# ratschlab/secedo

Measured on NVIDIA B200. Metric: similarity-matrix significant loci/s (8K cells, 0.5x), higher is better.
Workload: dtype int8 tensor-core counts (int32 accumulate) + f64 log-likelihood epilogue

## Files before the change

secedo_b200/csrc/common.cuh:

```cuda
#pragma once

#include <cuda_runtime.h>

#include <atomic>
#include <cstdarg>
#include <cstdint>
#include <cstdio>
#include <deque>
#include <map>
#include <string>
#include <unordered_map>
#include <vector>

#include "../../include/secedo_b200.h"

struct sgpu_ctx {
    int device = 0;
    int sm_count = 148;
    cudaStream_t own_stream = nullptr;
    cudaStream_t stream = nullptr;
    cudaStream_t copy_stream = nullptr;
    cudaStream_t d2h_stream = nullptr;
    cudaEvent_t out_done = nullptr;
    void *pending_out = nullptr;
// ... 199 lines not shown
    uint64_t slab_t0 = 0, slab_t1 = 0, slab_raw_tiles = 0;
    uint32_t slab_nb = 0;
    double *slab_raw = nullptr;
    unsigned long long *slab_minmax = nullptr;
    double *slab_out = nullptr;
};

constexpr uint32_t CODE_DROPPED = 0xFFFFFFFFu;
__host__ __device__ inline uint32_t code_cell(uint32_t c) { return c >> 4; }
__host__ __device__ inline uint32_t code_base(uint32_t c) { return (c >> 2) & 3u; }
__host__ __device__ inline bool code_tail(uint32_t c) { return (c >> 1) & 1u; }
__host__ __device__ inline bool code_multi(uint32_t c) { return c & 1u; }

struct LinkResult {
    DevBuf<uint32_t> sp_bits;
    DevBuf<uint64_t> sp_rank;
    DevBuf<uint32_t> sp_entry;
    DevBuf<uint32_t> sp_locus;
    DevBuf<uint32_t> sp_start;
    DevBuf<uint32_t> sp_head;
    DevBuf<uint32_t> sp_code;
    DevBuf<uint8_t> sp_drop;
    DevBuf<uint32_t> sp_rcode;
    DevBuf<uint64_t> g_off;
    DevBuf<uint32_t> g_list;
    DevBuf<uint8_t> g_base;
    DevBuf<uint32_t> g_nst;
    uint64_t n_special = 0;
    DevBuf<uint64_t> me_idx;
    DevBuf<uint32_t> me_code;
    DevBuf<uint32_t> me_locus;
    DevBuf<uint32_t> me_pos;
    DevBuf<uint32_t> me_beg;
    DevBuf<uint32_t> me_end;
    DevBuf<uint8_t> lchr;
    DevBuf<uint64_t> tail_locus;
    std::vector<uint64_t> h_tail_locus;
    DevBuf<uint32_t> tail_loci;
    uint64_t n_tail_loci = 0;
    DevBuf<uint32_t> gmap;
    uint32_t n_groups = 0, num_cells = 0;
    bool gmap_identity = false;
    bool ranged = false;
    DevBuf<uint8_t> owned;
    DevBuf<uint32_t> own_loci;
    uint64_t n_own = 0;
    DevBuf<uint32_t> code;
    uint64_t n_reads = 0, n_multi = 0, n_dropped = 0, n_tail = 0;
    uint64_t n_span_splits = 0;
};

int sgpu_scan_u8_u64(sgpu_ctx *ctx, const uint8_t *in, uint64_t *out, uint64_t n);
int sgpu_scan_u32_u64(sgpu_ctx *ctx, const uint32_t *in, uint64_t *out, uint64_t n);

int sgpu_filter_impl(sgpu_ctx *ctx, const sgpu_pileup *in, const uint32_t *h_id_to_pos, uint32_t n_groups,
                     double theta, int cell_proportion, sgpu_pileup **filtered, double *avg_coverage);
int sgpu_is_significant_impl(sgpu_ctx *ctx, const uint16_t *h_counts4, uint64_t n, double theta,
                             int cell_proportion, uint8_t *h_out);

struct RangeSpec {
    const uint32_t *own_pos_begin, *own_pos_end, *tail_position;
};
struct CutoffQuery {
    const uint8_t *whole;
    uint32_t *tail_position;
    uint8_t *resolved;
};
int sgpu_link_reads(sgpu_ctx *ctx, const sgpu_pileup *p, uint32_t num_cells, uint32_t L,
                    const uint32_t *h_group_id_to_pos, uint32_t n_groups, uint32_t num_threads,
                    LinkResult *out, const RangeSpec *range = nullptr, const CutoffQuery *cutq = nullptr);
int sgpu_cutoff_from_suffix(sgpu_ctx *ctx, const sgpu_pileup *p, uint32_t L, uint32_t num_threads, const uint8_t *h_whole,
                            uint32_t *h_tail_position, uint8_t *h_resolved);
int sgpu_link_dense_codes(sgpu_ctx *ctx, const sgpu_pileup *p, LinkResult *lr);
int sgpu_link_candidates(sgpu_ctx *ctx, LinkResult *lr, uint32_t min_nst);

int sgpu_choose_path(const sgpu_pileup *p, uint32_t num_cells);

int sgpu_scatter_pairs(sgpu_ctx *ctx, const sgpu_pileup *p, const LinkResult &lr, sgpu_counts *c,
                       int sign, bool only_tail_pairs, uint64_t *n_pairs);

int sgpu_multilocus(sgpu_ctx *ctx, const sgpu_pileup *p, LinkResult &lr, sgpu_counts *c,
                    uint32_t L, uint64_t *n_pairs_multi);

struct FTable {
    double F[SGPU_MAX_CLASS * SGPU_MAX_CLASS];
};
int sgpu_log_probs_impl(sgpu_ctx *ctx, double eps, double h, double theta, uint32_t L, uint32_t n,
                        double *h_ls, double *h_ld);
int sgpu_epilogue(sgpu_ctx *ctx, sgpu_counts *c, uint32_t L, double eps, double h, double theta,
                  int normalization, double *h_out, double **d_keep = nullptr, bool async_out = false);
int sgpu_output_wait_impl(sgpu_ctx *ctx);
int sgpu_slab_raw_impl(sgpu_ctx *ctx, sgpu_counts *c, const int32_t *const *peer_planes, const double *const *peer_spill,
                       uint32_t n_peers, uint32_t slab, uint32_t n_slabs, uint32_t L, double eps, double h, double theta,
                       double **d_extrema);
int sgpu_slab_finalize_impl(sgpu_ctx *ctx, sgpu_counts *c, int normalization, double *out, double **d_out);

int sgpu_em_impl(sgpu_ctx *ctx, const sgpu_pileup *p, const uint32_t *h_id_to_pos, uint32_t n_groups, double theta,
                 double *h_prob_b, uint32_t n_cells, uint32_t max_iterations, uint32_t *iterations, float *ms_total);

int sgpu_spectral_device(sgpu_ctx *ctx, const double *d_A, uint32_t n, uint32_t k, double tol, double *h_evals,
                         double *h_evecs, sgpu_spectral_stats *stats);
int sgpu_laplacian_device(sgpu_ctx *ctx, const double *d_A, uint32_t n, double *h_out);
int sgpu_spectral_matvec_host(sgpu_ctx *ctx, const double *h_M, uint32_t n, int width, const double *h_X, const double *h_W,
                              double alpha, double beta, double gamma, double *h_out);
int sgpu_build_gtable(sgpu_ctx *ctx, double eps, double h, double theta, uint32_t L, uint32_t n,
                      double *d_G , double *d_F );
// ... 24 lines not shown
```

secedo_b200/csrc/reads.cu:

```cuda
#include "common.cuh"

#include <algorithm>
#include <cstdlib>
#include <vector>

namespace {

constexpr int TB = 256;
constexpr uint64_t KEY_EMPTY = ~0ull;

__device__ __forceinline__ uint64_t mix64(uint64_t x) {
    x ^= x >> 33;
    x *= 0xff51afd7ed558ccdull;
    x ^= x >> 33;
    x *= 0xc4ceb9fe1a85ec53ull;
    x ^= x >> 33;
    return x;
}

__device__ __forceinline__ uint32_t chr_of_locus(const uint64_t *__restrict__ chr_ptr, uint32_t n_chr, uint64_t l) {
    uint32_t lo = 0, hi = n_chr;
    while (hi - lo > 1) {
        uint32_t mid = (lo + hi) >> 1;
        if (chr_ptr[mid] <= l) {
            lo = mid;
        } else {
            hi = mid;
        }
    }
    return lo;
}

__device__ __forceinline__ uint32_t locus_of_entry(const uint64_t *__restrict__ row_ptr, uint64_t n_loci, uint64_t e) {
    uint64_t lo = 0, hi = n_loci;
    while (hi - lo > 1) {
        const uint64_t mid = (lo + hi) >> 1;
        if (row_ptr[mid] <= e) {
            lo = mid;
        } else {
            hi = mid;
        }
    }
    return static_cast<uint32_t>(lo);
}

__global__ void __launch_bounds__(TB) locus_meta_kernel(const uint64_t *__restrict__ row_ptr,
                                                        const uint32_t *__restrict__ position,
                                                        const uint64_t *__restrict__ chr_ptr, uint32_t n_chr,
                                                        uint64_t n_loci, uint8_t *__restrict__ lchr,
                                                        unsigned int *__restrict__ max_row, int *__restrict__ err) {
    const uint64_t l = static_cast<uint64_t>(blockIdx.x) * TB + threadIdx.x;
    unsigned int n = 0;
    if (l < n_loci) {
        const uint32_t c = chr_of_locus(chr_ptr, n_chr, l);
        lchr[l] = static_cast<uint8_t>(c);
        if (l > chr_ptr[c] && position[l] <= position[l - 1]) {
            atomicExch(err, SGPU_E_POSITIONS);
        }
        n = static_cast<unsigned int>(min(row_ptr[l + 1] - row_ptr[l], static_cast<uint64_t>(0xFFFFFFFFu)));
    }
#pragma unroll
    for (int o = 16; o > 0; o >>= 1) {
        n = max(n, __shfl_xor_sync(0xffffffffu, n, o));
    }
    if ((threadIdx.x & 31) == 0 && n) {
        atomicMax(max_row, n);
    }
}

constexpr int WIN_THREADS = 512;
constexpr uint32_t SLOT_EMPTY = 0xFFFFu;
constexpr uint32_t REC_BUF = 1024;
constexpr uint32_t WIN_MAX_ENTRIES = 0xFFFEu;
constexpr size_t WIN_SMEM_LIMIT = 220 * 1024;

struct WinCounters {
    unsigned long long n_links;
};

__device__ __forceinline__ uint32_t slot_hash(uint32_t id, uint32_t shift) { return (id * 0x9E3779B1u) >> shift; }

__device__ __forceinline__ void emit_link(uint2 *rbuf, uint32_t *s_cnt, uint2 *__restrict__ links, uint64_t cap,
                                          WinCounters *__restrict__ ctr, uint32_t x, uint32_t y) {
    const uint32_t k = atomicAdd(s_cnt, 1u);
    if (k < REC_BUF) {
        rbuf[k] = make_uint2(x, y);
    } else {
        const unsigned long long g = atomicAdd(&ctr->n_links, 1ull);
        if (g < cap) {
            links[g] = make_uint2(x, y);
        }
    }
}

__device__ __forceinline__ void cp_async4(void *dst, const void *src) {
    asm volatile("cp.async.ca.shared.global [%0], [%1], 4;" ::"r"(static_cast<uint32_t>(__cvta_generic_to_shared(dst))), "l"(src) : "memory");
}
__device__ __forceinline__ void cp_async16(void *dst, const void *src) {
    asm volatile("cp.async.cg.shared.global [%0], [%1], 16;" ::"r"(static_cast<uint32_t>(__cvta_generic_to_shared(dst))), "l"(src) : "memory");
}
__device__ __forceinline__ void cp_async_commit() { asm volatile("cp.async.commit_group;" ::: "memory"); }
template <int N>
__device__ __forceinline__ void cp_async_wait() {
    asm volatile("cp.async.wait_group %0;" ::"n"(N) : "memory");
}

constexpr uint32_t WIN_RING = 3;
constexpr uint32_t WIN_META = 64;
constexpr uint32_t WIN_META_N = WIN_META + WIN_RING + 1;

__global__ void __launch_bounds__(WIN_THREADS, 2) link_window_kernel(
        const uint64_t *__restrict__ row_ptr, const uint32_t *__restrict__ position, const uint32_t *__restrict__ read_id,
        const uint64_t *__restrict__ src_off ,
        const uint8_t *__restrict__ lchr, uint64_t n_loci, uint32_t L, uint32_t loci_per_cta,
        uint32_t slots , uint32_t id_cap ,
        uint32_t n_ring ,
        uint2 *__restrict__ links, uint64_t cap, WinCounters *__restrict__ ctr) {
    extern __shared__ __align__(16) uint32_t s_mem[];
    uint32_t *ring = s_mem;
    uint2 *rbuf = reinterpret_cast<uint2 *>(s_mem + n_ring * id_cap);
    unsigned short *tab = reinterpret_cast<unsigned short *>(rbuf + REC_BUF);
    __shared__ uint64_t s_row[WIN_META_N + 1];
    __shared__ uint64_t s_src[WIN_META_N];
    __shared__ uint32_t s_pos[WIN_META_N];
    __shared__ uint8_t s_chr[WIN_META_N];
    __shared__ uint32_t s_cnt;
    __shared__ unsigned long long s_base;
    const uint32_t mask = slots - 1, shift = 32 - (31 - __clz(slots));
    const uint64_t la = static_cast<uint64_t>(blockIdx.x) * loci_per_cta;
    const uint64_t lb = min(n_loci, la + loci_per_cta);
    if (threadIdx.x == 0) {
        s_cnt = 0;
    }
    if (la >= lb) {
        return;
    }
    const bool aligned16 = (reinterpret_cast<uintptr_t>(read_id) & 15u) == 0;
    uint64_t meta0 = la;
    auto load_meta = [&](uint64_t base) {
        for (uint32_t i = threadIdx.x; i <= WIN_META_N; i += WIN_THREADS) {
            const uint64_t l = base + i;
            s_row[i] = row_ptr[min(l, n_loci)];
            if (i < WIN_META_N) {
                s_pos[i] = l < n_loci ? position[l] : 0;
                s_chr[i] = l < n_loci ? lchr[l] : 0xFF;
                s_src[i] = l < n_loci ? (src_off ? src_off[l] : row_ptr[l]) : 0;
            }
        }
    };
    auto prefetch = [&](uint64_t l) {
        if (l < n_loci && l - meta0 < WIN_META_N) {
            const uint64_t e0 = s_src[l - meta0];
            uint32_t *dst = ring + (l % n_ring) * id_cap + (e0 & 3u);
            const uint32_t *src = read_id + e0;
            const uint32_t n = static_cast<uint32_t>(s_row[l - meta0 + 1] - s_row[l - meta0]);
            const uint32_t head = aligned16 ? min(n, static_cast<uint32_t>((4 - (e0 & 3u)) & 3u)) : n;
            const uint32_t body = (n - head) >> 2;
            for (uint32_t i = threadIdx.x; i < head; i += WIN_THREADS) {
                cp_async4(dst + i, src + i);
            }
            for (uint32_t i = threadIdx.x; i < body; i += WIN_THREADS) {
                cp_async16(dst + head + 4 * i, src + head + 4 * i);
            }
            const uint32_t done = head + 4 * body;
// ... 192 lines not shown
    }
}

__global__ void __launch_bounds__(TB) ghash_emit_kernel(const uint64_t *__restrict__ row_ptr,
                                                        const uint32_t *__restrict__ read_id,
                                                        const uint8_t *__restrict__ lchr, uint64_t n_loci,
                                                        const uint64_t *__restrict__ keys, const uint32_t *__restrict__ vals,
                                                        uint64_t mask, uint2 *__restrict__ links, uint64_t cap,
                                                        WinCounters *__restrict__ ctr) {
    for (uint64_t l = blockIdx.x; l < n_loci; l += gridDim.x) {
        const uint64_t e0 = row_ptr[l], e1 = row_ptr[l + 1];
        const uint64_t chr = lchr[l];
        for (uint64_t base = e0; base < e1; base += TB) {
            const uint64_t e = base + threadIdx.x;
            uint32_t first = 0xFFFFFFFFu;
            if (e < e1) {
                const uint64_t key = (chr << 32) | read_id[e];
                uint64_t slot = mix64(key) & mask;
                while (keys[slot] != key) {
                    slot = (slot + 1) & mask;
                }
                first = vals[slot];
            }
            const bool hit = e < e1 && first != static_cast<uint32_t>(e);
            const uint32_t ballot = __ballot_sync(0xffffffffu, hit);
            if (ballot) {
                const int lane = threadIdx.x & 31, leader = __ffs(ballot) - 1;
                unsigned long long g = 0;
                if (lane == leader) {
                    g = atomicAdd(&ctr->n_links, static_cast<unsigned long long>(__popc(ballot)));
                }
                g = __shfl_sync(0xffffffffu, g, leader);
                if (hit) {
                    g += __popc(ballot & ((1u << lane) - 1u));
                    if (g < cap) {
                        links[g] = make_uint2(first, static_cast<uint32_t>(e));
                    }
                }
            }
        }
    }
}

__global__ void __launch_bounds__(TB) mark_kernel(const uint2 *__restrict__ links, uint64_t n_links,
                                                  uint32_t *__restrict__ bits) {
    const uint64_t i = static_cast<uint64_t>(blockIdx.x) * TB + threadIdx.x;
    if (i < n_links) {
        const uint2 r = links[i];
        atomicOr(&bits[r.x >> 5], 1u << (r.x & 31));
        atomicOr(&bits[r.y >> 5], 1u << (r.y & 31));
    }
}

__global__ void __launch_bounds__(TB) popc_kernel(const uint32_t *__restrict__ bits, uint64_t n_words,
                                                  uint32_t *__restrict__ pc) {
    const uint64_t w = static_cast<uint64_t>(blockIdx.x) * TB + threadIdx.x;
    if (w < n_words) {
        pc[w] = __popc(bits[w]);
    }
}

__device__ __forceinline__ uint32_t sid_of(const uint32_t *__restrict__ bits, const uint64_t *__restrict__ rank, uint32_t e) {
    return static_cast<uint32_t>(rank[e >> 5]) + __popc(bits[e >> 5] & ((1u << (e & 31)) - 1u));
}

__global__ void __launch_bounds__(TB) word_locus_kernel(const uint64_t *__restrict__ row_ptr, uint64_t n_loci,
                                                        uint64_t n_words, uint32_t *__restrict__ word_locus) {
    const int lane = threadIdx.x & 31;
    const uint64_t warps_total = static_cast<uint64_t>(gridDim.x) * (TB / 32);
    for (uint64_t l = static_cast<uint64_t>(blockIdx.x) * (TB / 32) + (threadIdx.x >> 5); l < n_loci; l += warps_total) {
        const uint64_t e0 = row_ptr[l], e1 = l + 1 < n_loci ? row_ptr[l + 1] : n_words * 32;
        for (uint64_t w = (e0 + 31) / 32 + lane; w * 32 < e1 && w < n_words; w += 32) {
            word_locus[w] = static_cast<uint32_t>(l);
        }
    }
}

__global__ void __launch_bounds__(TB) sp_list_kernel(const uint32_t *__restrict__ bits, const uint64_t *__restrict__ rank,
                                                     uint64_t n_words, const uint64_t *__restrict__ row_ptr,
                                                     const uint32_t *__restrict__ word_locus, uint32_t *__restrict__ sp_entry,
                                                     uint32_t *__restrict__ sp_first, uint32_t *__restrict__ sp_locus) {
    const uint64_t w = static_cast<uint64_t>(blockIdx.x) * TB + threadIdx.x;
    if (w >= n_words) {
        return;
    }
    uint32_t b = bits[w];
    if (b == 0) {
        return;
    }
    uint64_t k = rank[w];
    uint32_t l = word_locus[w];
    uint64_t l_end = row_ptr[l + 1];
    while (b) {
        const uint32_t bit = __ffs(b) - 1;
        b &= b - 1;
        const uint32_t e = static_cast<uint32_t>(w * 32 + bit);
        while (e >= l_end) {
            ++l;
            l_end = row_ptr[l + 1];
        }
        sp_entry[k] = e;
        sp_first[k] = e;
        sp_locus[k] = l;
        ++k;
    }
}

__global__ void __launch_bounds__(TB) link_min_kernel(const uint2 *__restrict__ links, uint64_t n_links,
                                                      const uint32_t *__restrict__ bits, const uint64_t *__restrict__ rank,
                                                      uint32_t *__restrict__ sp_first, int *__restrict__ changed) {
    const uint64_t i = static_cast<uint64_t>(blockIdx.x) * TB + threadIdx.x;
    if (i >= n_links) {
        return;
    }
    const uint2 r = links[i];
    const uint32_t sx = sid_of(bits, rank, r.x), sy = sid_of(bits, rank, r.y);
    const uint32_t fx = sp_first[sx], fy = sp_first[sy];
    const uint32_t m = min(fx, fy);
    if (fx != m) {
        atomicMin(&sp_first[sx], m);
        *changed = 1;
    }
    if (fy != m) {
        atomicMin(&sp_first[sy], m);
// ... 327 lines not shown
        s_multi = 0;
    }
    __syncthreads();
    uint32_t dropped = 0, multi_head = 0;
    for (uint64_t s = static_cast<uint64_t>(blockIdx.x) * TB + threadIdx.x; s < n_special; s += static_cast<uint64_t>(gridDim.x) * TB) {
        const uint32_t h = sp_head[s];
        const uint32_t multi = g_nst[h] >= 2 ? 1u : 0u;
        multi_head += (h == s) & multi;
        const bool drop = sp_drop[s] != 0;
        if (drop) {
            sp_code[s] = CODE_DROPPED;
            ++dropped;
        }
        if (!drop || h == s) {
            const uint32_t gid = gid_base[sp_entry[h]] >> 2;
            uint32_t cell = 0;
            if (gid >= n_groups || (cell = gmap[gid]) >= num_cells) {
                atomicExch(err, SGPU_E_CELL_RANGE);
                cell = 0;
            }
            const uint32_t base = gid_base[sp_entry[s]] & 3u;
            const uint32_t hl = sp_locus[h];
            const uint32_t tail = hl >= tail_locus[lchr[hl]] ? 1u : 0u;
            if (!drop) {
                sp_code[s] = (cell << 4) | (base << 2) | (tail << 1) | multi;
            }
            if (h == s) {
                sp_rcode[s] = (cell << 4) | (tail << 1) | multi;
            }
        }
    }
#pragma unroll
    for (int o = 16; o > 0; o >>= 1) {
        dropped += __shfl_xor_sync(0xffffffffu, dropped, o);
        multi_head += __shfl_xor_sync(0xffffffffu, multi_head, o);
    }
    if ((threadIdx.x & 31) == 0) {
        if (dropped) {
            atomicAdd(&s_dropped, dropped);
        }
        if (multi_head) {
            atomicAdd(&s_multi, multi_head);
        }
    }
    __syncthreads();
    if (threadIdx.x == 0) {
        if (s_dropped) {
            atomicAdd(&stats[0], static_cast<unsigned long long>(s_dropped));
        }
        if (s_multi) {
            atomicAdd(&stats[1], static_cast<unsigned long long>(s_multi));
        }
    }
}

__global__ void __launch_bounds__(TB) sp_start_kernel(const uint32_t *__restrict__ sp_locus, uint64_t n_special,
                                                      uint64_t n_loci, uint32_t *__restrict__ sp_start) {
    const uint64_t l = static_cast<uint64_t>(blockIdx.x) * TB + threadIdx.x;
    if (l > n_loci) {
        return;
    }
    uint64_t lo = 0, hi = n_special;
    while (lo < hi) {
        const uint64_t mid = (lo + hi) >> 1;
        if (sp_locus[mid] < l) {
            lo = mid + 1;
        } else {
            hi = mid;
        }
    }
    sp_start[l] = static_cast<uint32_t>(lo);
}

__global__ void __launch_bounds__(TB) me_flag_kernel(const uint32_t *__restrict__ sp_code, const uint32_t *__restrict__ sp_head,
                                                     const uint32_t *__restrict__ sp_locus, const uint64_t *__restrict__ g_off,
                                                     const uint32_t *__restrict__ g_list, const uint32_t *__restrict__ g_nst,
                                                     uint64_t n_special, uint32_t min_nst, uint32_t *__restrict__ flag,
                                                     uint32_t *__restrict__ pos) {
    const uint64_t s = static_cast<uint64_t>(blockIdx.x) * TB + threadIdx.x;
    if (s >= n_special) {
        return;
    }
    const uint32_t c = sp_code[s];
    uint32_t f = 0;
    if (c != CODE_DROPPED && (c & 1u) && g_nst[sp_head[s]] >= min_nst) {
        const uint32_t h = sp_head[s], loc = sp_locus[s], n = g_nst[h];
        const uint64_t o = g_off[h];
        uint32_t i = 0;
        while (i < n && g_list[o + i] != loc) {
            ++i;
        }
        f = i + 1 < n ? 1u : 0u;
        pos[s] = static_cast<uint32_t>(o + i);
    }
    flag[s] = f;
}

__global__ void __launch_bounds__(TB) me_compact_kernel(const uint32_t *__restrict__ flag, const uint32_t *__restrict__ pos,
                                                        const uint64_t *__restrict__ me_idx, const uint32_t *__restrict__ sp_code,
                                                        const uint32_t *__restrict__ sp_head, const uint32_t *__restrict__ sp_locus,
                                                        const uint64_t *__restrict__ g_off, const uint32_t *__restrict__ g_nst,
                                                        uint64_t n_special, uint32_t *__restrict__ me_code,
                                                        uint32_t *__restrict__ me_locus, uint32_t *__restrict__ me_pos,
                                                        uint32_t *__restrict__ me_beg, uint32_t *__restrict__ me_end) {
    const uint64_t s = static_cast<uint64_t>(blockIdx.x) * TB + threadIdx.x;
    if (s >= n_special || !flag[s]) {
        return;
    }
    const uint64_t k = me_idx[s];
    const uint32_t h = sp_head[s];
    me_code[k] = sp_code[s];
    me_locus[k] = sp_locus[s];
    me_pos[k] = pos[s];
    me_beg[k] = static_cast<uint32_t>(g_off[h]);
    me_end[k] = static_cast<uint32_t>(g_off[h]) + g_nst[h];
}

template <typename GB>
__global__ void __launch_bounds__(TB) dense_codes_kernel(const uint64_t *__restrict__ row_ptr,
                                                         const GB *__restrict__ gid_base,
                                                         const uint8_t *__restrict__ lchr,
                                                         const uint64_t *__restrict__ tail_locus,
                                                         const uint32_t *__restrict__ gmap, uint32_t n_groups,
                                                         uint32_t num_cells, uint64_t n_loci, uint32_t *__restrict__ code,
// ... 64 lines not shown
            SGPU_CUDA(ctx, cudaMemcpyAsync(out->tail_locus.p, p->d_chr_ptr + 1, p->n_chr * sizeof(uint64_t), cudaMemcpyDeviceToDevice, st));
        }
        SGPU_CUDA(ctx, out->tail_loci.alloc(1, ctx));
        return SGPU_OK;
    }

    SGPU_TRACE(ctx, "link: enter");
    DevBuf<int> d_err;
    DevBuf<unsigned int> d_maxn;
    DevBuf<WinCounters> d_ctr;
    DevBuf<unsigned long long> d_stats;
    DevBuf<uint64_t> readbase, n_tail_reads;
    SGPU_CUDA(ctx, d_err.alloc(2, ctx));
    SGPU_CUDA(ctx, d_maxn.alloc(1, ctx));
    SGPU_CUDA(ctx, d_ctr.alloc(1, ctx));
    SGPU_CUDA(ctx, d_stats.alloc(2, ctx));
    SGPU_CUDA(ctx, readbase.alloc(P + 1, ctx));
    SGPU_CUDA(ctx, n_tail_reads.alloc(p->n_chr, ctx));
    SGPU_CUDA(ctx, cudaMemsetAsync(d_err.p, 0, 2 * sizeof(int), st));
    SGPU_CUDA(ctx, cudaMemsetAsync(d_maxn.p, 0, sizeof(unsigned int), st));
    SGPU_CUDA(ctx, cudaMemsetAsync(d_ctr.p, 0, sizeof(WinCounters), st));
    SGPU_CUDA(ctx, cudaMemsetAsync(d_stats.p, 0, 2 * sizeof(unsigned long long), st));

    SGPU_LAUNCH(ctx, (locus_meta_kernel<<<blocks_for(P), TB, 0, st>>>(p->d_row_ptr, p->d_position, p->d_chr_ptr, p->n_chr, P,
                                                                       out->lchr.p, d_maxn.p, d_err.p)));
    uint32_t max_n = p->max_row;
    if (max_n == 0) {
        SGPU_CUDA(ctx, cudaMemcpyAsync(&ctx->h_scratch[0], d_maxn.p, sizeof(unsigned int), cudaMemcpyDeviceToHost, st));
        SGPU_CUDA(ctx, cudaStreamSynchronize(st));
        max_n = static_cast<uint32_t>(ctx->h_scratch[0] & 0xFFFFFFFFu);
        p->max_row = max_n;
    }

    SGPU_TRACE(ctx, "link: allocs+meta");
    const uint32_t id_cap = (max_n + 3 + 3) & ~3u;
    unsigned long long slot_factor = 3;
    if (const char *env = getenv("SECEDO_B200_WIN_SLOT_FACTOR")) {
        slot_factor = static_cast<unsigned long long>(std::max(1, atoi(env)));
    }
    const size_t win_limit = ctx->win_smem_limit ? std::min<size_t>(ctx->win_smem_limit, WIN_SMEM_LIMIT) : WIN_SMEM_LIMIT;
    auto pow2_slots = [&](unsigned long long want) {
        uint32_t sl = 1024;
        while (sl < want && sl < 65536) {
            sl <<= 1;
        }
        return sl;
    };
    uint32_t n_ring = WIN_RING, slots = 1024;
    auto win_smem = [&](uint32_t s) {
        return static_cast<size_t>(n_ring) * id_cap * 4 + REC_BUF * sizeof(uint2) + static_cast<size_t>(s) * 2;
    };
    auto choose_geometry = [&](size_t limit) {
        const uint32_t s_full = pow2_slots(slot_factor * max_n), s_half = std::min(s_full, pow2_slots(2ull * max_n));
        const uint32_t cand[4][2] = { { WIN_RING, s_full }, { 2, s_full }, { WIN_RING, s_half }, { 2, s_half } };
        const char *env_ring = getenv("SECEDO_B200_WIN_RING");
        for (const auto &cd : cand) {
            n_ring = cd[0];
            slots = cd[1];
            if (win_smem(slots) <= limit && !(env_ring && env_ring[0] == '1')) {
                return true;
            }
        }
        n_ring = 1;
        slots = s_full;
        while (slots > 1024 && win_smem(slots) > limit) {
            slots >>= 1;
        }
        return win_smem(slots) <= limit && 4ull * slots >= 5ull * max_n;
    };
    bool window_fits = choose_geometry(win_limit);
    if (!window_fits && win_limit < WIN_SMEM_LIMIT) {
        window_fits = choose_geometry(WIN_SMEM_LIMIT);
    }
    const char *force_global = getenv("SECEDO_B200_FORCE_GLOBAL_HASH");
    const bool use_window = max_n <= WIN_MAX_ENTRIES && window_fits && 4ull * slots >= 5ull * max_n
            && !(force_global && force_global[0] == '1');
    const unsigned locus_grid = static_cast<unsigned>(std::min<uint64_t>(P, static_cast<uint64_t>(ctx->sm_count) * 16));

    DevBuf<uint2> links;
    uint64_t cap = std::max<uint64_t>(E / 8, 4096);
    uint64_t NL = 0;
    for (int attempt = 0; attempt < 2; ++attempt) {
        SGPU_CUDA(ctx, links.alloc(cap, ctx));
        SGPU_CUDA(ctx, cudaMemsetAsync(d_ctr.p, 0, sizeof(WinCounters), st));
        if (use_window) {
            const size_t smem = win_smem(slots);
            SGPU_CUDA(ctx, cudaFuncSetAttribute(link_window_kernel, cudaFuncAttributeMaxDynamicSharedMemorySize, static_cast<int>(smem)));
            const unsigned per_sm = static_cast<unsigned>(std::max<size_t>(1, std::min<size_t>(4, (224 * 1024) / (smem + 2560))));
            const uint64_t want = std::min<uint64_t>(P, static_cast<uint64_t>(ctx->sm_count) * per_sm);
            const uint32_t loci_per_cta = static_cast<uint32_t>(ceil_div_u64(P, want));
            const unsigned wgrid = static_cast<unsigned>(ceil_div_u64(P, loci_per_cta));
            SGPU_TRY(sgpu_cache_preference(ctx, false));
            SGPU_LAUNCH(ctx, (link_window_kernel<<<wgrid, WIN_THREADS, smem, st>>>(p->d_row_ptr, p->d_position,
                                                                                  p->d_read_id ? p->d_read_id : p->view_read_id,
                                                                                  p->d_read_id ? nullptr : p->view_off, out->lchr.p, P, L,
                                                                                  loci_per_cta, slots, id_cap, n_ring, links.p, cap, d_ctr.p)));
        } else {
            SGPU_TRY(sgpu_pileup_materialize(ctx, p));
            DevBuf<uint64_t> keys;
            DevBuf<uint32_t> vals;
            uint64_t hcap = 1024;
            while (hcap < 2 * E) {
                hcap <<= 1;
            }
            SGPU_CUDA(ctx, keys.alloc(hcap, ctx));
            SGPU_CUDA(ctx, vals.alloc(hcap, ctx));
            SGPU_CUDA(ctx, cudaMemsetAsync(keys.p, 0xFF, hcap * sizeof(uint64_t), st));
            SGPU_CUDA(ctx, cudaMemsetAsync(vals.p, 0xFF, hcap * sizeof(uint32_t), st));
            SGPU_LAUNCH(ctx, (ghash_insert_kernel<<<locus_grid, TB, 0, st>>>(p->d_row_ptr, p->d_read_id, out->lchr.p, P, keys.p, vals.p, hcap - 1)));
            SGPU_LAUNCH(ctx, (ghash_emit_kernel<<<locus_grid, TB, 0, st>>>(p->d_row_ptr, p->d_read_id, out->lchr.p, P, keys.p, vals.p, hcap - 1,
                                                                            links.p, cap, d_ctr.p)));
        }
        SGPU_CUDA(ctx, cudaGetLastError());
        if (ctx->flush_point == 0) {
            SGPU_TRY(sgpu_tensor_flush(ctx, true));
        }
        SGPU_CUDA(ctx, cudaMemcpyAsync(&ctx->h_scratch[0], d_ctr.p, sizeof(uint64_t), cudaMemcpyDeviceToHost, st));
        SGPU_CUDA(ctx, cudaStreamSynchronize(st));
        NL = ctx->h_scratch[0];
        if (NL <= cap) {
            break;
        }
        if (attempt == 1) {
            return sgpu_fail(ctx, SGPU_E_CUDA, "link list overflow on retry (%llu > %llu)", (unsigned long long)NL, (unsigned long long)cap);
        }
        cap = NL;
    }

    SGPU_TRACE(ctx, "link: window kernel");
    uint64_t NS = 0;
    DevBuf<uint32_t> nf_locus;
    DevBuf<uint64_t> nf_scan;
    if (NL) {
        DevBuf<uint32_t> pc;
        SGPU_CUDA(ctx, pc.alloc(W, ctx));
        SGPU_CUDA(ctx, out->sp_rank.alloc(W + 1, ctx));
        SGPU_LAUNCH(ctx, (mark_kernel<<<blocks_for(NL), TB, 0, st>>>(links.p, NL, out->sp_bits.p)));
        SGPU_LAUNCH(ctx, (popc_kernel<<<blocks_for(W), TB, 0, st>>>(out->sp_bits.p, W, pc.p)));
        SGPU_TRY(sgpu_scan_u32_u64(ctx, pc.p, out->sp_rank.p, W));
        SGPU_CUDA(ctx, cudaMemcpyAsync(&ctx->h_scratch[0], out->sp_rank.p + W, sizeof(uint64_t), cudaMemcpyDeviceToHost, st));
        SGPU_CUDA(ctx, cudaStreamSynchronize(st));
        NS = ctx->h_scratch[0];
    }
    SGPU_TRACE(ctx, "link: mark+rank");
    out->n_special = NS;
    SGPU_CUDA(ctx, out->sp_start.alloc(P + 1, ctx));
    if (NS == 0) {
        SGPU_CUDA(ctx, cudaMemsetAsync(out->sp_start.p, 0, (P + 1) * sizeof(uint32_t), st));
    }
    DevBuf<uint32_t> sp_first, g_cnt, cursor;
    if (NS) {
        SGPU_CUDA(ctx, out->sp_entry.alloc(NS, ctx));
        SGPU_CUDA(ctx, out->sp_locus.alloc(NS, ctx));
        SGPU_CUDA(ctx, out->sp_head.alloc(NS, ctx));
        SGPU_CUDA(ctx, out->sp_code.alloc(NS, ctx));
        SGPU_CUDA(ctx, out->sp_drop.alloc(NS, ctx));
        SGPU_CUDA(ctx, out->sp_rcode.alloc(NS, ctx));
        SGPU_CUDA(ctx, out->g_off.alloc(NS + 1, ctx));
        SGPU_CUDA(ctx, out->g_list.alloc(NS, ctx));
        SGPU_CUDA(ctx, out->g_base.alloc(NS, ctx));
        SGPU_CUDA(ctx, out->g_nst.alloc(NS, ctx));
        SGPU_CUDA(ctx, sp_first.alloc(NS, ctx));
        SGPU_CUDA(ctx, g_cnt.alloc(NS, ctx));
        SGPU_CUDA(ctx, cursor.alloc(NS, ctx));
        SGPU_CUDA(ctx, nf_locus.alloc(P, ctx));
        SGPU_CUDA(ctx, nf_scan.alloc(P + 1, ctx));
        {
            DevBuf<uint32_t> word_locus;
            SGPU_CUDA(ctx, word_locus.alloc(W, ctx));
            SGPU_LAUNCH(ctx, (word_locus_kernel<<<locus_grid, TB, 0, st>>>(p->d_row_ptr, P, W, word_locus.p)));
            SGPU_LAUNCH(ctx, (sp_list_kernel<<<blocks_for(W), TB, 0, st>>>(out->sp_bits.p, out->sp_rank.p, W, p->d_row_ptr, word_locus.p,
                                                                            out->sp_entry.p, sp_first.p, out->sp_locus.p)));
        }
        SGPU_LAUNCH(ctx, (sp_start_kernel<<<blocks_for(P + 1), TB, 0, st>>>(out->sp_locus.p, NS, P, out->sp_start.p)));
    }
    auto build_reads = [&](bool careful) -> int {
        if (NS == 0) {
            return SGPU_OK;
        }
        SGPU_CUDA(ctx, cudaMemsetAsync(g_cnt.p, 0, NS * sizeof(uint32_t), st));
        SGPU_CUDA(ctx, cudaMemsetAsync(cursor.p, 0, NS * sizeof(uint32_t), st));
        SGPU_CUDA(ctx, cudaMemsetAsync(out->g_nst.p, 0, NS * sizeof(uint32_t), st));
        SGPU_CUDA(ctx, cudaMemsetAsync(out->sp_drop.p, 0, NS, st));
        if (!careful) {
            for (int sweep = 0; sweep < 3; ++sweep) {
                SGPU_LAUNCH(ctx, (link_min_kernel<<<blocks_for(NL), TB, 0, st>>>(links.p, NL, out->sp_bits.p, out->sp_rank.p, sp_first.p,
                                                                                 d_err.p + 1)));
                if (sweep == 1) {
                    SGPU_CUDA(ctx, cudaMemsetAsync(d_err.p + 1, 0, sizeof(int), st));
                }
            }
        } else {
            SGPU_CUDA(ctx, cudaMemcpyAsync(sp_first.p, out->sp_entry.p, NS * sizeof(uint32_t), cudaMemcpyDeviceToDevice, st));
            for (int sweep = 0;; ++sweep) {
                SGPU_CUDA(ctx, cudaMemsetAsync(d_err.p + 1, 0, sizeof(int), st));
                SGPU_LAUNCH(ctx, (link_min_kernel<<<blocks_for(NL), TB, 0, st>>>(links.p, NL, out->sp_bits.p, out->sp_rank.p, sp_first.p,
                                                                                 d_err.p + 1)));
                SGPU_CUDA(ctx, cudaMemcpyAsync(&ctx->h_scratch[0], d_err.p + 1, sizeof(int), cudaMemcpyDeviceToHost, st));
                SGPU_CUDA(ctx, cudaStreamSynchronize(st));
                if (static_cast<int>(ctx->h_scratch[0] & 0xFFFFFFFFu) == 0) {
                    break;
                }
                if (sweep > 100000) {
                    return sgpu_fail(ctx, SGPU_E_FRAGMENT_SPAN, "read linking did not settle");
                }
            }
        }
        auto group = [&]() -> int {
            SGPU_LAUNCH(ctx, (group_count_kernel<<<blocks_for(NS), TB, 0, st>>>(out->sp_bits.p, out->sp_rank.p, sp_first.p, NS, out->sp_head.p, g_cnt.p)));
            SGPU_TRY(sgpu_scan_u32_u64(ctx, g_cnt.p, out->g_off.p, NS));
            SGPU_LAUNCH(ctx, (group_fill_kernel<<<blocks_for(NS), TB, 0, st>>>(out->sp_head.p, out->sp_locus.p, out->g_off.p, NS, cursor.p,
                                                                               out->g_list.p)));
            return SGPU_OK;
        };
        SGPU_TRY(group());
        if (careful) {
            DevBuf<unsigned long long> d_splits;
            SGPU_CUDA(ctx, d_splits.alloc(1, ctx));
            SGPU_CUDA(ctx, cudaMemsetAsync(d_splits.p, 0, sizeof(unsigned long long), st));
            SGPU_LAUNCH(ctx, (split_span_kernel<<<blocks_for(NS), TB, 0, st>>>(out->sp_head.p, out->sp_entry.p, out->sp_locus.p, out->g_off.p, NS,
                                                                               out->g_list.p, p->d_position, L, sp_first.p, d_splits.p)));
            SGPU_CUDA(ctx, cudaMemcpyAsync(&ctx->h_scratch[0], d_splits.p, sizeof(uint64_t), cudaMemcpyDeviceToHost, st));
            SGPU_CUDA(ctx, cudaStreamSynchronize(st));
            out->n_span_splits = ctx->h_scratch[0];
            SGPU_CUDA(ctx, cudaMemsetAsync(g_cnt.p, 0, NS * sizeof(uint32_t), st));
            SGPU_CUDA(ctx, cudaMemsetAsync(cursor.p, 0, NS * sizeof(uint32_t), st));
            SGPU_TRY(group());
// ... 245 lines not shown
```

secedo_b200/csrc/scan.cu:

```cuda
#include "common.cuh"

namespace {

constexpr int SCAN_THREADS = 512;
constexpr int SCAN_ITEMS = 8;
constexpr int SCAN_TILE = SCAN_THREADS * SCAN_ITEMS;

__device__ __forceinline__ uint64_t warp_incl_scan(uint64_t v, int lane) {
#pragma unroll
    for (int o = 1; o < 32; o <<= 1) {
        uint64_t t = __shfl_up_sync(0xffffffffu, v, o);
        if (lane >= o) {
            v += t;
        }
    }
    return v;
}

__device__ __forceinline__ uint64_t block_excl_scan(uint64_t v, uint64_t *total) {
    __shared__ uint64_t warp_sums[SCAN_THREADS / 32];
    const int lane = threadIdx.x & 31, warp = threadIdx.x >> 5;
    uint64_t incl = warp_incl_scan(v, lane);
    if (lane == 31) {
        warp_sums[warp] = incl;
    }
    __syncthreads();
    if (warp == 0) {
        uint64_t w = lane < SCAN_THREADS / 32 ? warp_sums[lane] : 0;
        uint64_t wi = warp_incl_scan(w, lane);
        if (lane < SCAN_THREADS / 32) {
            warp_sums[lane] = wi - w;
        }
        if (lane == SCAN_THREADS / 32 - 1) {
            *total = wi;
        }
    }
    __syncthreads();
    uint64_t r = warp_sums[warp] + incl - v;
    __syncthreads();
    return r;
}

template <typename T>
__global__ void __launch_bounds__(SCAN_THREADS) scan_reduce_kernel(const T *__restrict__ in, uint64_t n,
                                                                  uint64_t *__restrict__ block_sums) {
    __shared__ uint64_t total;
    const uint64_t base = static_cast<uint64_t>(blockIdx.x) * SCAN_TILE;
    uint64_t s = 0;
#pragma unroll
    for (int k = 0; k < SCAN_ITEMS; ++k) {
        uint64_t i = base + static_cast<uint64_t>(k) * SCAN_THREADS + threadIdx.x;
        if (i < n) {
            s += in[i];
        }
    }
    block_excl_scan(s, &total);
    if (threadIdx.x == 0) {
        block_sums[blockIdx.x] = total;
    }
}

__global__ void __launch_bounds__(SCAN_THREADS) scan_sums_kernel(uint64_t *__restrict__ block_sums, uint64_t nb,
                                                                uint64_t *__restrict__ grand) {
    __shared__ uint64_t total;
    uint64_t carry = 0;
    for (uint64_t base = 0; base < nb; base += SCAN_THREADS) {
        uint64_t i = base + threadIdx.x;
        uint64_t v = i < nb ? block_sums[i] : 0;
        uint64_t ex = block_excl_scan(v, &total);
        if (i < nb) {
            block_sums[i] = carry + ex;
        }
        carry += total;
        __syncthreads();
    }
    if (threadIdx.x == 0) {
        *grand = carry;
    }
}

template <typename T>
__global__ void __launch_bounds__(SCAN_THREADS) scan_apply_kernel(const T *__restrict__ in, uint64_t n,
                                                                 const uint64_t *__restrict__ block_sums,
                                                                 uint64_t *__restrict__ out) {
    __shared__ uint64_t total;
    const uint64_t base = static_cast<uint64_t>(blockIdx.x) * SCAN_TILE + static_cast<uint64_t>(threadIdx.x) * SCAN_ITEMS;
    uint64_t v[SCAN_ITEMS];
    uint64_t s = 0;
    if (sizeof(T) == 1 && SCAN_ITEMS == 8 && base + SCAN_ITEMS <= n && (reinterpret_cast<uintptr_t>(in) & 7) == 0) {
        const uint64_t w = *reinterpret_cast<const uint64_t *>(in + base);
#pragma unroll
        for (int k = 0; k < SCAN_ITEMS; ++k) {
            v[k] = (w >> (8 * k)) & 0xFF;
            s += v[k];
        }
    } else {
#pragma unroll
        for (int k = 0; k < SCAN_ITEMS; ++k) {
            uint64_t i = base + k;
            v[k] = i < n ? static_cast<uint64_t>(in[i]) : 0;
            s += v[k];
        }
    }
    uint64_t ex = block_excl_scan(s, &total) + block_sums[blockIdx.x];
#pragma unroll
    for (int k = 0; k < SCAN_ITEMS; ++k) {
        uint64_t i = base + k;
        if (i < n) {
            out[i] = ex;
        }
        ex += v[k];
    }
}

template <typename T>
int scan_impl(sgpu_ctx *ctx, const T *in, uint64_t *out, uint64_t n) {
    cudaStream_t st = ctx->stream;
    if (n == 0) {
        SGPU_CUDA(ctx, cudaMemsetAsync(out, 0, sizeof(uint64_t), st));
        return SGPU_OK;
    }
    const uint64_t nb = ceil_div_u64(n, SCAN_TILE);
    DevBuf<uint64_t> sums;
    SGPU_CUDA(ctx, sums.alloc(nb, ctx));
    SGPU_LAUNCH(ctx, (scan_reduce_kernel<T><<<static_cast<unsigned>(nb), SCAN_THREADS, 0, st>>>(in, n, sums.p)));
    SGPU_LAUNCH(ctx, (scan_sums_kernel<<<1, SCAN_THREADS, 0, st>>>(sums.p, nb, out + n)));
    SGPU_LAUNCH(ctx, (scan_apply_kernel<T><<<static_cast<unsigned>(nb), SCAN_THREADS, 0, st>>>(in, n, sums.p, out)));
    SGPU_CUDA(ctx, cudaGetLastError());
    return SGPU_OK;
}

}

int sgpu_scan_u8_u64(sgpu_ctx *ctx, const uint8_t *in, uint64_t *out, uint64_t n) {
    return scan_impl<uint8_t>(ctx, in, out, n);
}

int sgpu_scan_u32_u64(sgpu_ctx *ctx, const uint32_t *in, uint64_t *out, uint64_t n) {
    return scan_impl<uint32_t>(ctx, in, out, n);
}
```

Measured before the change: 7.506 million.

## Fuse popcount into rank scan, fold sp_start into locus kernel, allow 3 window CTAs per SM

The read-linking path now counts bits inside the scan kernels, which removes a separate popcount kernel and its temporary buffer. The sp_start binary search moves into the word-locus kernel, computed per locus directly from the bit rank. The link window kernel targets 3 CTAs per SM: its record buffer is halved, launch bounds and carveout are raised, and geometries that fit 73KB smem are preferred. The trade-off is more register and smem pressure and more global atomic spills from the smaller record buffer. A profiling script for the link kernels is also added.

```diff
diff --git a/profiles/link_probe.py b/profiles/link_probe.py
--- /dev/null
+++ b/profiles/link_probe.py
@@ -0,0 +1,84 @@
+import argparse
+import json
+import os
+import statistics
+import subprocess
+import sys
+
+ROOT = os.path.dirname(os.path.dirname(os.path.abspath(__file__)))
+sys.path.insert(0, ROOT)
+
+LINK_KERNELS = ("locus_meta", "link_window", "ghash", "mark_kernel", "scan_", "locus_sp", "sp_list", "link_min", "group_",
+                "nonfirst", "split_span", "mate_rule", "readbase", "cutoff", "sp_finish", "me_flag", "me_compact")
+
+
+def run(iters: int, trace_dir: str) -> dict:
+    import numpy as np
+    import bench
+    from secedo_b200 import api
+    w = bench.WORKLOAD
+    ctx = api.Context(0)
+    N = w["n_cells"]
+    ident = np.arange(N, dtype=np.uint32)
+    raw = ctx.synth_pileup(N, w["coverage"], w["n_chr"], w["loci_per_chr"], n_clones=w["n_clones"], frac_somatic=w["frac_somatic"],
+                           frac_germline=w["frac_germline"], theta=w["theta"], spacing=w["spacing"], p_multi=w["p_multi"],
+                           p_mate=w["p_mate"], p_mate_mismatch=w["p_mate_mismatch"], seed=1000)
+    flt = api.Filter(w["theta"], 4, ctx)
+    counts = api.Counts(ctx, N)
+
+    def one():
+        f, _ = flt.filter_device(raw, ident)
+        counts.zero()
+        st = counts.accumulate(f, w["L"], ident, w["eps"], w["h"], w["theta"], 8, "auto")
+        f.free()
+        counts.finalize(w["L"], w["eps"], w["h"], w["theta"], "ADD_MIN", to_host=False)
+        return st
+
+    for _ in range(2):
+        one()
+    ctx.synchronize()
+    stats = [one() for _ in range(iters)]
+    ctx.synchronize()
+    out = {k: statistics.median(s[k] for s in stats) for k in stats[0] if k.startswith("ms_")}
+    if trace_dir:
+        import torch
+        from torch.profiler import ProfilerActivity, profile
+        with profile(activities=[ProfilerActivity.CUDA]) as prof:
+            one()
+            ctx.synchronize()
+            torch.cuda.synchronize()
+        rows = {}
+        for ev in prof.events():
+            if ev.device_type.name == "CUDA" and any(k in ev.name for k in LINK_KERNELS):
+                n, t = rows.get(ev.name, (0, 0.0))
+                rows[ev.name] = (n + 1, t + ev.device_time_total)
+        os.makedirs(trace_dir, exist_ok=True)
+        with open(os.path.join(trace_dir, "link_kernels.txt"), "w") as fh:
+            total = sum(t for _, t in rows.values())
+            fh.write(f"read-linking kernels of one sub-batch (torch.profiler), sum {total:.1f} us\n")
+            for name, (n, t) in sorted(rows.items(), key=lambda kv: -kv[1][1]):
+                fh.write(f"{t:9.1f} us {n:3d}  {name[:110]}\n")
+        out["trace_sum_us"] = total
+    return out
+
+
+def main() -> None:
+    ap = argparse.ArgumentParser()
+    ap.add_argument("--iters", type=int, default=8)
+    ap.add_argument("--trace", metavar="OUT_DIR")
+    ap.add_argument("--child", action="store_true", help=argparse.SUPPRESS)
+    a = ap.parse_args()
+    if a.child:
+        print(json.dumps(run(a.iters, a.trace)))
+        return
+    for mode, env in (("alone", {"SECEDO_B200_ASYNC_GEMM": "0"}), ("live", {})):
+        args = [sys.executable, "-B", os.path.abspath(__file__), "--child", "--iters", str(a.iters)]
+        if a.trace and mode == "alone":
+            args += ["--trace", a.trace]
+        r = subprocess.run(args, env={**os.environ, **env}, capture_output=True, text=True, check=True)
+        res = json.loads(r.stdout.strip().splitlines()[-1])
+        print(mode, json.dumps({k: round(v, 3) for k, v in res.items()}), flush=True)
+
+
+if __name__ == "__main__":
+    main()
diff --git a/secedo_b200/csrc/common.cuh b/secedo_b200/csrc/common.cuh
--- a/secedo_b200/csrc/common.cuh
+++ b/secedo_b200/csrc/common.cuh
@@ -275,6 +275,7 @@
 
 int sgpu_scan_u8_u64(sgpu_ctx *ctx, const uint8_t *in, uint64_t *out, uint64_t n);
 int sgpu_scan_u32_u64(sgpu_ctx *ctx, const uint32_t *in, uint64_t *out, uint64_t n);
+int sgpu_scan_popc_u64(sgpu_ctx *ctx, const uint32_t *bits, uint64_t *out, uint64_t n);
 
 int sgpu_filter_impl(sgpu_ctx *ctx, const sgpu_pileup *in, const uint32_t *h_id_to_pos, uint32_t n_groups,
                      double theta, int cell_proportion, sgpu_pileup **filtered, double *avg_coverage);
diff --git a/secedo_b200/csrc/reads.cu b/secedo_b200/csrc/reads.cu
--- a/secedo_b200/csrc/reads.cu
+++ b/secedo_b200/csrc/reads.cu
@@ -70,9 +70,11 @@
 
 constexpr int WIN_THREADS = 512;
 constexpr uint32_t SLOT_EMPTY = 0xFFFFu;
-constexpr uint32_t REC_BUF = 1024;
+constexpr uint32_t REC_BUF = 512;
 constexpr uint32_t WIN_MAX_ENTRIES = 0xFFFEu;
 constexpr size_t WIN_SMEM_LIMIT = 220 * 1024;
+constexpr size_t WIN_SMEM_3CTA = 73 * 1024;
+constexpr unsigned WIN_CTAS_PER_SM = 3;
 
 struct WinCounters {
     unsigned long long n_links;
@@ -109,7 +111,7 @@
 constexpr uint32_t WIN_META = 64;
 constexpr uint32_t WIN_META_N = WIN_META + WIN_RING + 1;
 
-__global__ void __launch_bounds__(WIN_THREADS, 2) link_window_kernel(
+__global__ void __launch_bounds__(WIN_THREADS, WIN_CTAS_PER_SM) link_window_kernel(
         const uint64_t *__restrict__ row_ptr, const uint32_t *__restrict__ position, const uint32_t *__restrict__ read_id,
         const uint64_t *__restrict__ src_off ,
         const uint8_t *__restrict__ lchr, uint64_t n_loci, uint32_t L, uint32_t loci_per_cta,
@@ -408,24 +410,25 @@
     }
 }
 
-__global__ void __launch_bounds__(TB) popc_kernel(const uint32_t *__restrict__ bits, uint64_t n_words,
-                                                  uint32_t *__restrict__ pc) {
-    const uint64_t w = static_cast<uint64_t>(blockIdx.x) * TB + threadIdx.x;
-    if (w < n_words) {
-        pc[w] = __popc(bits[w]);
-    }
-}
-
 __device__ __forceinline__ uint32_t sid_of(const uint32_t *__restrict__ bits, const uint64_t *__restrict__ rank, uint32_t e) {
     return static_cast<uint32_t>(rank[e >> 5]) + __popc(bits[e >> 5] & ((1u << (e & 31)) - 1u));
 }
 
-__global__ void __launch_bounds__(TB) word_locus_kernel(const uint64_t *__restrict__ row_ptr, uint64_t n_loci,
-                                                        uint64_t n_words, uint32_t *__restrict__ word_locus) {
+__global__ void __launch_bounds__(TB) locus_sp_kernel(const uint64_t *__restrict__ row_ptr, uint64_t n_loci,
+                                                      uint64_t n_words, const uint32_t *__restrict__ bits,
+                                                      const uint64_t *__restrict__ rank, uint32_t *__restrict__ word_locus,
+                                                      uint32_t *__restrict__ sp_start) {
     const int lane = threadIdx.x & 31;
     const uint64_t warps_total = static_cast<uint64_t>(gridDim.x) * (TB / 32);
-    for (uint64_t l = static_cast<uint64_t>(blockIdx.x) * (TB / 32) + (threadIdx.x >> 5); l < n_loci; l += warps_total) {
-        const uint64_t e0 = row_ptr[l], e1 = l + 1 < n_loci ? row_ptr[l + 1] : n_words * 32;
+    for (uint64_t l = static_cast<uint64_t>(blockIdx.x) * (TB / 32) + (threadIdx.x >> 5); l <= n_loci; l += warps_total) {
+        const uint64_t e0 = row_ptr[l];
+        if (lane == 0) {
+            sp_start[l] = sid_of(bits, rank, static_cast<uint32_t>(e0));
+        }
+        if (l == n_loci) {
+            break;
+        }
+        const uint64_t e1 = l + 1 < n_loci ? row_ptr[l + 1] : n_words * 32;
         for (uint64_t w = (e0 + 31) / 32 + lane; w * 32 < e1 && w < n_words; w += 32) {
             word_locus[w] = static_cast<uint32_t>(l);
         }
@@ -859,24 +862,6 @@
             atomicAdd(&stats[1], static_cast<unsigned long long>(s_multi));
         }
     }
-}
-
-__global__ void __launch_bounds__(TB) sp_start_kernel(const uint32_t *__restrict__ sp_locus, uint64_t n_special,
-                                                      uint64_t n_loci, uint32_t *__restrict__ sp_start) {
-    const uint64_t l = static_cast<uint64_t>(blockIdx.x) * TB + threadIdx.x;
-    if (l > n_loci) {
-        return;
-    }
-    uint64_t lo = 0, hi = n_special;
-    while (lo < hi) {
-        const uint64_t mid = (lo + hi) >> 1;
-        if (sp_locus[mid] < l) {
-            lo = mid + 1;
-        } else {
-            hi = mid;
-        }
-    }
-    sp_start[l] = static_cast<uint32_t>(lo);
 }
 
 __global__ void __launch_bounds__(TB) me_flag_kernel(const uint32_t *__restrict__ sp_code, const uint32_t *__restrict__ sp_head,
@@ -1047,12 +1032,13 @@
     };
     auto choose_geometry = [&](size_t limit) {
         const uint32_t s_full = pow2_slots(slot_factor * max_n), s_half = std::min(s_full, pow2_slots(2ull * max_n));
-        const uint32_t cand[4][2] = { { WIN_RING, s_full }, { 2, s_full }, { WIN_RING, s_half }, { 2, s_half } };
+        const uint32_t cand[6][3] = { { WIN_RING, s_full, 1 }, { 2, s_full, 1 },
+                                      { WIN_RING, s_full, 0 }, { 2, s_full, 0 }, { WIN_RING, s_half, 0 }, { 2, s_half, 0 } };
         const char *env_ring = getenv("SECEDO_B200_WIN_RING");
         for (const auto &cd : cand) {
             n_ring = cd[0];
             slots = cd[1];
-            if (win_smem(slots) <= limit && !(env_ring && env_ring[0] == '1')) {
+            if (win_smem(slots) <= (cd[2] ? std::min(limit, WIN_SMEM_3CTA) : limit) && !(env_ring && env_ring[0] == '1')) {
                 return true;
             }
         }
@@ -1081,7 +1067,8 @@
         if (use_window) {
             const size_t smem = win_smem(slots);
             SGPU_CUDA(ctx, cudaFuncSetAttribute(link_window_kernel, cudaFuncAttributeMaxDynamicSharedMemorySize, static_cast<int>(smem)));
-            const unsigned per_sm = static_cast<unsigned>(std::max<size_t>(1, std::min<size_t>(4, (224 * 1024) / (smem + 2560))));
+            SGPU_CUDA(ctx, cudaFuncSetAttribute(link_window_kernel, cudaFuncAttributePreferredSharedMemoryCarveout, cudaSharedmemCarveoutMaxShared));
+            const unsigned per_sm = static_cast<unsigned>(std::max<size_t>(1, std::min<size_t>(WIN_CTAS_PER_SM, (224 * 1024) / (smem + 2560))));
             const uint64_t want = std::min<uint64_t>(P, static_cast<uint64_t>(ctx->sm_count) * per_sm);
             const uint32_t loci_per_cta = static_cast<uint32_t>(ceil_div_u64(P, want));
             const unsigned wgrid = static_cast<unsigned>(ceil_div_u64(P, loci_per_cta));
@@ -1127,12 +1114,9 @@
     DevBuf<uint32_t> nf_locus;
     DevBuf<uint64_t> nf_scan;
     if (NL) {
-        DevBuf<uint32_t> pc;
-        SGPU_CUDA(ctx, pc.alloc(W, ctx));
         SGPU_CUDA(ctx, out->sp_rank.alloc(W + 1, ctx));
         SGPU_LAUNCH(ctx, (mark_kernel<<<blocks_for(NL), TB, 0, st>>>(links.p, NL, out->sp_bits.p)));
-        SGPU_LAUNCH(ctx, (popc_kernel<<<blocks_for(W), TB, 0, st>>>(out->sp_bits.p, W, pc.p)));
-        SGPU_TRY(sgpu_scan_u32_u64(ctx, pc.p, out->sp_rank.p, W));
+        SGPU_TRY(sgpu_scan_popc_u64(ctx, out->sp_bits.p, out->sp_rank.p, W));
         SGPU_CUDA(ctx, cudaMemcpyAsync(&ctx->h_scratch[0], out->sp_rank.p + W, sizeof(uint64_t), cudaMemcpyDeviceToHost, st));
         SGPU_CUDA(ctx, cudaStreamSynchronize(st));
         NS = ctx->h_scratch[0];
@@ -1163,11 +1147,11 @@
         {
             DevBuf<uint32_t> word_locus;
             SGPU_CUDA(ctx, word_locus.alloc(W, ctx));
-            SGPU_LAUNCH(ctx, (word_locus_kernel<<<locus_grid, TB, 0, st>>>(p->d_row_ptr, P, W, word_locus.p)));
+            SGPU_LAUNCH(ctx, (locus_sp_kernel<<<locus_grid, TB, 0, st>>>(p->d_row_ptr, P, W, out->sp_bits.p, out->sp_rank.p, word_locus.p,
+                                                                          out->sp_start.p)));
             SGPU_LAUNCH(ctx, (sp_list_kernel<<<blocks_for(W), TB, 0, st>>>(out->sp_bits.p, out->sp_rank.p, W, p->d_row_ptr, word_locus.p,
                                                                             out->sp_entry.p, sp_first.p, out->sp_locus.p)));
         }
-        SGPU_LAUNCH(ctx, (sp_start_kernel<<<blocks_for(P + 1), TB, 0, st>>>(out->sp_locus.p, NS, P, out->sp_start.p)));
     }
     auto build_reads = [&](bool careful) -> int {
         if (NS == 0) {
diff --git a/secedo_b200/csrc/scan.cu b/secedo_b200/csrc/scan.cu
--- a/secedo_b200/csrc/scan.cu
+++ b/secedo_b200/csrc/scan.cu
@@ -41,7 +41,16 @@
     return r;
 }
 
-template <typename T>
+template <bool POPC, typename T>
+__device__ __forceinline__ uint64_t scan_value(T x) {
+    if constexpr (POPC) {
+        return static_cast<uint64_t>(__popc(x));
+    } else {
+        return static_cast<uint64_t>(x);
+    }
+}
+
+template <typename T, bool POPC>
 __global__ void __launch_bounds__(SCAN_THREADS) scan_reduce_kernel(const T *__restrict__ in, uint64_t n,
                                                                   uint64_t *__restrict__ block_sums) {
     __shared__ uint64_t total;
@@ -51,7 +60,7 @@
     for (int k = 0; k < SCAN_ITEMS; ++k) {
         uint64_t i = base + static_cast<uint64_t>(k) * SCAN_THREADS + threadIdx.x;
         if (i < n) {
-            s += in[i];
+            s += scan_value<POPC>(in[i]);
         }
     }
     block_excl_scan(s, &total);
@@ -79,7 +88,7 @@
     }
 }
 
-template <typename T>
+template <typename T, bool POPC>
 __global__ void __launch_bounds__(SCAN_THREADS) scan_apply_kernel(const T *__restrict__ in, uint64_t n,
                                                                  const uint64_t *__restrict__ block_sums,
                                                                  uint64_t *__restrict__ out) {
@@ -98,7 +107,7 @@
 #pragma unroll
         for (int k = 0; k < SCAN_ITEMS; ++k) {
             uint64_t i = base + k;
-            v[k] = i < n ? static_cast<uint64_t>(in[i]) : 0;
+            v[k] = i < n ? scan_value<POPC>(in[i]) : 0;
             s += v[k];
         }
     }
@@ -113,7 +122,7 @@
     }
 }
 
-template <typename T>
+template <typename T, bool POPC = false>
 int scan_impl(sgpu_ctx *ctx, const T *in, uint64_t *out, uint64_t n) {
     cudaStream_t st = ctx->stream;
     if (n == 0) {
@@ -123,9 +132,9 @@
     const uint64_t nb = ceil_div_u64(n, SCAN_TILE);
     DevBuf<uint64_t> sums;
     SGPU_CUDA(ctx, sums.alloc(nb, ctx));
-    SGPU_LAUNCH(ctx, (scan_reduce_kernel<T><<<static_cast<unsigned>(nb), SCAN_THREADS, 0, st>>>(in, n, sums.p)));
+    SGPU_LAUNCH(ctx, (scan_reduce_kernel<T, POPC><<<static_cast<unsigned>(nb), SCAN_THREADS, 0, st>>>(in, n, sums.p)));
     SGPU_LAUNCH(ctx, (scan_sums_kernel<<<1, SCAN_THREADS, 0, st>>>(sums.p, nb, out + n)));
-    SGPU_LAUNCH(ctx, (scan_apply_kernel<T><<<static_cast<unsigned>(nb), SCAN_THREADS, 0, st>>>(in, n, sums.p, out)));
+    SGPU_LAUNCH(ctx, (scan_apply_kernel<T, POPC><<<static_cast<unsigned>(nb), SCAN_THREADS, 0, st>>>(in, n, sums.p, out)));
     SGPU_CUDA(ctx, cudaGetLastError());
     return SGPU_OK;
 }
@@ -139,3 +148,7 @@
 int sgpu_scan_u32_u64(sgpu_ctx *ctx, const uint32_t *in, uint64_t *out, uint64_t n) {
     return scan_impl<uint32_t>(ctx, in, out, n);
 }
+
+int sgpu_scan_popc_u64(sgpu_ctx *ctx, const uint32_t *bits, uint64_t *out, uint64_t n) {
+    return scan_impl<uint32_t, true>(ctx, bits, out, n);
+}
```

New measurement: 7.557 million, median of 6. About the same (+0.7%).
